# DCDmllm/AnyEdit

Hardware: AMD Instinct MI355X
Metric: edited-images/sec @512x512, 50 DDIM steps (higher is better)
Workload: dtype bf16; 1 GPU; configs[1]: AnySD (SD-1.5 UNet in=8 + task embedding/expert adapters) 512x512 bf16, 50 DDIM steps, batch=4/GPU, 3-branch CFG (UNet batch 12); images_per_gpu=4, ddim_steps=50, cfg_branches=3, hip_graph=True, parallelism=dp1 (image-sharded, no data-path collective)

## Files before the change

### anyedit_amd/_lib.py

```python
import ctypes
import os

import torch

_HERE = os.path.dirname(os.path.abspath(__file__))
LIB_PATH = os.environ.get("AE_LIB_PATH") or os.path.join(_HERE, "libanyedit_hip.so")

c_void_p, c_int, c_long, c_float = ctypes.c_void_p, ctypes.c_int, ctypes.c_long, ctypes.c_float

SIGNATURES = {
    "ae_version": [],
    "ae_last_error": [],
    "ae_device_arch": [ctypes.c_char_p, c_int],
    "ae_device_info": [ctypes.POINTER(c_int), ctypes.POINTER(c_long), ctypes.POINTER(c_int)],
    "ae_gemm_bf16": [c_void_p, c_long, c_void_p, c_long, c_int, c_void_p, c_long, c_void_p, c_long, c_int, c_int, c_int,
                     c_void_p, c_void_p, c_long, c_void_p, c_long, c_int, c_int, c_int, c_void_p, c_void_p],
    "ae_conv3x3_workspace_floats": [c_int, c_int, c_int, c_int, c_int, c_int, c_int],
    "ae_conv3x3_partials_bf16": [c_void_p, c_void_p, c_int, c_int, c_int, c_int, c_int, c_void_p, c_int, c_void_p, c_void_p],
    "ae_groupnorm_splitk_supported": [c_int, c_int, c_int, c_int, c_int],
    "ae_groupnorm_splitk_nhwc_bf16": [c_void_p, c_int, c_void_p, c_void_p, c_long, c_void_p, c_void_p, c_void_p, c_int, c_int, c_int, c_int, c_float, c_int, c_void_p],
    "ae_conv3x3_bf16": [c_void_p, c_void_p, c_void_p, c_void_p, c_long, c_void_p, c_void_p, c_int, c_int, c_int, c_int, c_int,
                        c_int, c_int, c_int, c_void_p, c_void_p, c_int, c_void_p],
    "ae_conv3x3_up2_bf16": [c_void_p, c_void_p, c_void_p, c_void_p, c_int, c_int, c_int, c_int, c_int, c_void_p, c_void_p],
    "ae_groupnorm_rows_per_chunk": [c_int, c_int],
    "ae_groupnorm_workspace_floats": [c_int, c_int, c_int, c_int],
    "ae_groupnorm_nhwc_bf16": [c_void_p, c_void_p, c_int, c_void_p, c_void_p, c_void_p, c_int, c_int, c_int, c_int, c_float,
                               c_int, c_void_p, c_void_p, c_void_p, c_void_p, c_void_p, c_void_p],
    "ae_layernorm_bf16": [c_void_p, c_void_p, c_void_p, c_void_p, c_int, c_int, c_float, c_void_p],
    "ae_attn_fwd_bf16": [c_void_p, c_void_p, c_void_p, c_void_p, c_int, c_int, c_int, c_int, c_int,
                         c_long, c_long, c_long, c_long, c_long, c_long, c_long, c_long, c_long, c_long, c_long, c_long,
                         c_float, c_void_p, c_void_p, c_int, c_int, c_void_p, c_void_p, c_int,
                         c_void_p, c_void_p, c_int, c_long, c_long, c_long, c_long, c_long, c_long, c_void_p, c_void_p, c_void_p,
                         c_void_p],
    "ae_attn_bwd_bf16": [c_void_p] * 10 + [c_int] * 5 + [c_long] * 21 + [c_float, c_void_p, c_int, c_void_p, c_void_p],
    "ae_attn_bwd_workspace_floats": [c_int] * 5,
    "ae_groupnorm_bwd_workspace_floats": [c_int, c_int, c_int, c_int],
    "ae_groupnorm_bwd_nhwc_bf16": [c_void_p, c_void_p, c_int, c_void_p, c_void_p, c_void_p, c_void_p, c_void_p, c_int, c_int, c_int,
                                   c_int, c_float, c_int, c_void_p, c_void_p, c_void_p, c_int, c_void_p],
    "ae_layernorm_bwd_bf16": [c_void_p, c_void_p, c_void_p, c_void_p, c_void_p, c_int, c_int, c_float, c_int, c_void_p],
    "ae_layernorm_param_grad_f32": [c_void_p, c_void_p, c_void_p, c_void_p, c_void_p, c_int, c_int, c_void_p],
    "ae_add_bf16": [c_void_p, c_void_p, c_void_p, c_long, c_void_p],
    "ae_axpy_bf16": [c_void_p, c_void_p, c_float, c_void_p, c_long, c_void_p],
    "ae_geglu_fwd_bf16": [c_void_p, c_void_p, c_long, c_int, c_void_p],
    "ae_geglu_bwd_bf16": [c_void_p, c_void_p, c_void_p, c_long, c_int, c_void_p],
    "ae_sumpool2x2_bf16": [c_void_p, c_void_p, c_int, c_int, c_int, c_int, c_void_p],
# ... 56 lines not shown
                             c_float, c_void_p],
    "ae_layernorm_act_bf16": [c_void_p, c_void_p, c_void_p, c_void_p, c_long, c_int, c_float, c_int, c_void_p],
    "ae_sam_pe_encode_f32": [c_void_p, c_void_p, c_void_p, c_void_p, c_void_p, c_int, c_int, c_float, c_float, c_float, c_void_p],
    "ae_sam_mask_downscale_bf16": [c_void_p] * 10 + [c_int, c_int, c_int, c_float, c_void_p],
    "ae_sam_mask_product_f32": [c_void_p, c_void_p, c_void_p, c_int, c_int, c_int, c_int, c_int, c_void_p],
    "ae_sam_postprocess_masks": [c_void_p, c_void_p, c_void_p] + [c_int] * 8 + [c_float, c_int, c_void_p],
    "ae_nms_sorted_f32": [c_void_p, c_void_p, c_int, c_float, c_void_p],
    "ae_sam_preprocess_f32": [c_void_p, c_int, c_void_p, c_int, c_int, c_int, c_int, c_int, c_void_p, c_void_p, c_void_p],
    "ae_patchify_f32_bf16": [c_void_p, c_void_p, c_int, c_int, c_int, c_int, c_int, c_void_p],
    "ae_mse_f32": [c_void_p, c_void_p, c_void_p, c_long, c_void_p],
    "ae_lincomb4_f32": [c_void_p, c_void_p, c_float, c_void_p, c_float, c_void_p, c_float, c_void_p, c_float, c_long, c_void_p],
    "ae_dpm_adaptive_err_f32": [c_void_p, c_void_p, c_void_p, c_float, c_float, c_int, c_long, c_void_p, c_void_p],
    "ae_task_gate": [c_void_p, c_void_p, c_void_p, c_void_p, c_int, c_int, c_int, c_int, c_void_p, c_void_p, c_void_p, c_void_p],
    "ae_attn_causal_short_bf16": [c_void_p, c_void_p, c_void_p, c_void_p, c_int, c_int, c_int, c_int] + [c_long] * 12 + [c_float, c_void_p],
    "ae_clip_embed_bf16": [c_void_p, c_int, c_void_p, c_void_p, c_void_p, c_int, c_int, c_int, c_int, c_int, c_void_p],
    "ae_bias_act_f32_bf16": [c_void_p, c_long, c_void_p, c_void_p, c_long, c_long, c_int, c_int, c_void_p],
    "ae_clip_pool_eos_bf16": [c_void_p, c_int, c_void_p, c_void_p, c_int, c_int, c_int, c_long, c_void_p],
    "ae_clip_patch_rows_bf16": [c_void_p, c_int, c_void_p, c_int, c_int, c_int, c_int, c_int, c_int, c_float, c_void_p, c_void_p, c_void_p],
    "ae_clip_vision_embed_ln_bf16": [c_void_p, c_long, c_void_p, c_void_p, c_void_p, c_void_p, c_void_p, c_int, c_int, c_int, c_float, c_void_p],
    "ae_clip_vision_pool_ln_bf16": [c_void_p, c_long, c_void_p, c_void_p, c_void_p, c_int, c_int, c_float, c_void_p],
    "ae_dino_embed_bf16": [c_void_p, c_long, c_void_p, c_void_p, c_void_p, c_void_p, c_int, c_int, c_int, c_void_p],
    "ae_swiglu_f32_bf16": [c_void_p, c_long, c_void_p, c_void_p, c_long, c_long, c_int, c_void_p],
}
_RESTYPES = {"ae_last_error": ctypes.c_char_p, "ae_groupnorm_workspace_floats": c_long, "ae_conv3x3_workspace_floats": c_long,
             "ae_groupnorm_bwd_workspace_floats": c_long, "ae_attn_fp8_workspace_bytes": c_long, "ae_attn_bwd_workspace_floats": c_long,
             "ae_xattn_fused_kv_bytes": c_long}


class AnyEditHipError(RuntimeError):
    pass


def _load():
    if not os.path.exists(LIB_PATH):
        raise ImportError(
            f"{LIB_PATH} is missing: the HIP extension is REQUIRED (no CPU/eager fallback exists). "
            "Build it with `python -c 'import __graft_entry__ as g; g.build()'` or `python anyedit_amd/build.py`.")
    lib = ctypes.CDLL(LIB_PATH)
    for name, argtypes in SIGNATURES.items():
        fn = getattr(lib, name)
        fn.argtypes = argtypes
        fn.restype = _RESTYPES.get(name, c_int)
    return lib


lib = _load()

# ... 12 lines not shown
```

### anyedit_amd/csrc/gemm_conv.hip

```cpp
#include "common.hpp"
#include <stdlib.h>
#include <type_traits>

namespace {

#ifndef AE_CONV_SPEC
#define AE_CONV_SPEC 1
#endif
#ifndef AE_GEMM_WA_DEFAULT
#define AE_GEMM_WA_DEFAULT 3
#endif
#ifndef AE_GEMM_PP_DEFAULT
#define AE_GEMM_PP_DEFAULT 63
#endif
#ifndef AE_XE_OCC
#define AE_XE_OCC 4
#endif
#ifndef AE_PP_LAB
#define AE_PP_LAB 0
#endif
#ifndef AE_PP_PRIO
#define AE_PP_PRIO 1
#endif
#ifndef AE_PP_DMA_FIRST
// ... 10 lines not shown
    const bf16_t* W;
    void* C;
    const float* bias;
    const bf16_t* res;
    const float* addvec;
    int M, N, K, Ksplit;
    long lda, lda2, ldw, ldc, ldr, ldav;
    int epi, out_f32, rows_per_batch;
    int H, Wd, Cin, CinPad, Ho, Wo, stride, ups;
    unsigned a_bytes, a2_bytes, w_bytes;
    int splitk;
    float* partial;
    float* colstats;
    int kmajor;
    int m_fast;
    int xe;
    float* rowstats;
    const float* ln_stats;
    const float* ln_colsum;
    int ln_parts;
    float ln_eps;
    int sub2;
    int defer_reduce;
};

__device__ __forceinline__ void lds_dma16(__amdgpu_buffer_rsrc_t rs, bf16_t* lds_dst, int voffset, int soffset = 0) {
#if defined(__HIP_DEVICE_COMPILE__)
    __builtin_amdgcn_raw_ptr_buffer_load_lds(rs, (__attribute__((address_space(3))) void*)lds_dst, 16, voffset, soffset, 0, 0);
#endif
}

#ifdef AE_GEMM_LAB
__device__ unsigned long long g_gemm_dbg[32];
#define GL_T(i) do { const unsigned long long t_ = __builtin_readcyclecounter(); if (lab_me) g_gemm_dbg[lab_base + (i)] += t_ - tlast; tlast = t_; } while (0)
#elif defined(AE_GEMM_TRACE)
constexpr int TR_K0 = 18, TR_T = 6;
__device__ unsigned long long g_pp_trace[8 * TR_T * 16];
#define GL_T(i) do { __builtin_amdgcn_sched_barrier(0); tr_t[(i)] = __builtin_readcyclecounter(); __builtin_amdgcn_sched_barrier(0); } while (0)
#else
#define GL_T(i)
#endif

constexpr int epilogue_passes(int FM, int bytes_per_frag_row, int lds_bytes) {
    for (int ps = 1; ps <= FM; ++ps)
        if (FM % ps == 0 && (FM / ps) * bytes_per_frag_row <= lds_bytes) return ps;
    return FM;
// ... 101 lines not shown
                for (int t9 = 0; t9 < 9; ++t9) {
                    const int iy = iy0 + t9 / 3, ix = ix0 + t9 % 3;
                    if ((unsigned)iy < (unsigned)Hv && (unsigned)ix < (unsigned)Wv && (p.ups != 2 || ((iy | ix) & 1) == 0)) fa_mask[i] |= 1u << t9;
                }
            }

        }
    }
#pragma unroll
    for (int i = 0; i < B_CH; ++i) {
        const int id = tid + i * NT, row = id >> 3;
        const int c = GLDS ? ((id & 7) ^ (row & 7)) : (id & 7);
        fb_off[i] = (n0 + row < p.N) ? (int)((long)(n0 + row) * p.ldw * 2) + c * 16 : OOB;
    }
    const bool conv_fast = (AMODE == A_CONV3) && p.Cin == p.CinPad;

    u32x4 ra[A_CH], rb[B_CH];
    const u32x4 zero4 = {0u, 0u, 0u, 0u};
    const int KT_all = (p.K + BK - 1) / BK;
    const int kt_per = (KT_all + p.splitk - 1) / p.splitk;
    const int kt_begin = (AMODE == A_CONV3 && p.sub2) ? 0 : split * kt_per;
    const int KT = max(min(KT_all - kt_begin, kt_per), 0);
    const int klast = p.K - 8;
    const int conv_per = AMODE == A_CONV3 ? p.CinPad / BK : 1;
    const unsigned conv_per_magic = (AE_CONV_SPEC && conv_per > 1) ? 0xFFFFFFFFu / (unsigned)conv_per + 1u : 0u;
    const unsigned pp_magic = (WA == 3 && conv_per > 1) ? 0xFFFFFFFFu / (unsigned)conv_per + 1u : 0u;
    int ld_tap = (kt_begin * BK) / (AMODE == A_CONV3 ? p.CinPad : 1 << 30), ld_ci = (AMODE == A_CONV3) ? (kt_begin * BK) % p.CinPad : 0;
    if (AMODE == A_CONV3 && p.kmajor) { ld_tap = kt_begin % 9; ld_ci = (kt_begin / 9) * BK; }

    auto load_tile = [&](int kt) __attribute__((always_inline)) {
        const int k0 = (kt_begin + kt) * BK;
        const bool full_k = k0 + BK <= p.K;
        if (AMODE == A_DENSE && full_k && (k0 + BK <= p.Ksplit || k0 >= p.Ksplit)) {
            if (k0 < p.Ksplit) {
#pragma unroll
                for (int i = 0; i < A_CH; ++i) ra[i] = __builtin_amdgcn_raw_buffer_load_b128(rsA, fa_off[i] + k0 * 2, 0, 0);
            } else {
#pragma unroll
                for (int i = 0; i < A_CH; ++i) ra[i] = __builtin_amdgcn_raw_buffer_load_b128(rsA2, fa2_off[i] + (k0 - p.Ksplit) * 2, 0, 0);
            }
#pragma unroll
            for (int i = 0; i < B_CH; ++i) rb[i] = __builtin_amdgcn_raw_buffer_load_b128(rsW, fb_off[i] + k0 * 2, 0, 0);
            return;
        }
        if (conv_fast) {
            const int ky = ld_tap / 3, kx = ld_tap - ky * 3;
// ... 168 lines not shown
        auto dma_a = [&](int kt, int buf) __attribute__((always_inline)) {
            const int fs = WA == 2 ? buf : 0;
            const int k0 = (kt_begin + kt) * BK;
            if (AMODE == A_DENSE) {
                const bool second = k0 >= p.Ksplit;
                if (AE_CONV_SPEC) {
                    if (!second) {
#pragma unroll
                        for (int i = 0; i < A_CH; ++i) lds_dma16(rsA, sA + buf * BM * BK + (wave + (NT / 64) * i) * 8 * BK, fa_off[i], k0 * 2);
                    } else {
#pragma unroll
                        for (int i = 0; i < A_CH; ++i) lds_dma16(rsA2, sA + buf * BM * BK + (wave + (NT / 64) * i) * 8 * BK, fa2_off[i], (k0 - p.Ksplit) * 2);
                    }
                } else {
#pragma unroll
                for (int i = 0; i < A_CH; ++i) {
                    bf16_t* dst = sA + buf * BM * BK + (wave + (NT / 64) * i) * 8 * BK;
                    if (!second) lds_dma16(rsA, dst, fa_off[i], k0 * 2);
                    else lds_dma16(rsA2, dst, fa2_off[i], (k0 - p.Ksplit) * 2);
                }
                }
            } else {
                constexpr bool KM1 = AE_CONV_SPEC && WA == 2;
                int cur_tap = ld_tap, cur_ci = ld_ci;
                constexpr bool STATELESS = true;
                if (STATELESS) {
                    const int lin = kt_begin + kt;
                    if (KM1 || p.kmajor) { cur_tap = lin % 9; cur_ci = (lin / 9) * BK; }
                    else if (AE_CONV_SPEC) {
                        cur_tap = conv_per == 1 ? lin : (int)__umulhi((unsigned)lin, conv_per_magic);
                        cur_ci = (lin - cur_tap * conv_per) * BK;
                    } else { const int per = p.CinPad / BK; cur_tap = lin / per; cur_ci = (lin - cur_tap * per) * BK; }
                }
                const int ky = (!KM1 && p.sub2) ? py + (cur_tap >> 1) : cur_tap / 3, kx = (!KM1 && p.sub2) ? px + (cur_tap & 1) : cur_tap - ky * 3;
                const int mbit = (!KM1 && p.sub2) ? ky * 3 + kx : cur_tap;
                if (cur_ci == 0 || kt == 0 || KM1 || p.kmajor || WA == 2) {
#pragma unroll
                    for (int i = 0; i < A_CH; ++i) {
                        int src = fa_off[i] + ((ky * p.Wd + kx) * p.Cin) * 2;
                        if (!KM1 && p.ups) {
                            const int cc = ((tid + i * NT) & 7) ^ (((tid + i * NT) >> 3) & 7);
                            src = (int)((a_base[i] + (long)(max(a_iy[i] + ky, 0) >> 1) * p.Wd + (max(a_ix[i] + kx, 0) >> 1)) * p.Cin + cc * 8) * 2;
                        }
                        fa_cur[fs][i] = ((fa_mask[i] >> mbit) & 1u) ? src : OOB;
                    }
                }
// ... 853 lines not shown
    hipLaunchKernelGGL(kern, dim3(grid), dim3(threads), lds, stream, a);
    return ae_check_launch(what);
}

template <int AMODE>
int launch(const GemmArgs& a_in, hipStream_t stream) {
    GemmArgs a = a_in;
    static const int mfast_env = getenv("AE_GEMM_MFAST") ? atoi(getenv("AE_GEMM_MFAST")) : -1;
    a.m_fast = mfast_env >= 0 ? mfast_env : (AMODE == A_CONV3 ? (9L * a.N >= 8L * a.M) : ((long)a.N >= 3L * a.M)) ? 1 : 0;
    const int cand[4][2] = {{128, 128}, {128, 64}, {64, 64}, {128, 160}};
    static const int t160 = getenv("AE_GEMM_T160") ? atoi(getenv("AE_GEMM_T160")) : 1;
    int pick = a.splitk > 1 ? 0 : pick_tile(a.M, a.N);
    static const int force_tile = getenv("AE_GEMM_TILE") ? atoi(getenv("AE_GEMM_TILE")) : -1;
    if (force_tile >= 0 && force_tile <= 2 && a.splitk <= 1) pick = force_tile;
    if (pick == 3 && (!t160 || AMODE == A_DENSE || a.epi == EPI_GEGLU || a.splitk > 1)) pick = 1;
    static const int w8 = getenv("AE_GEMM_W8") ? atoi(getenv("AE_GEMM_W8")) : 2;
    static const int wk_knob = getenv("AE_GEMM_WK") ? atoi(getenv("AE_GEMM_WK")) : 0;
    const int kt_block = ((a.K + BK - 1) / BK + a.splitk - 1) / a.splitk;
    const bool wk_env = wk_knob == 2 || (wk_knob == 1 && AMODE == A_CONV3 && kt_block >= 60);
    const bool conv = AMODE == A_CONV3;
    const char* what = conv ? "ae_conv3x3_bf16" : "ae_gemm_bf16";
    static const int glds_env = getenv("AE_GEMM_GLDS") ? atoi(getenv("AE_GEMM_GLDS")) : 1;
    const bool glds = glds_env && (conv ? (a.Cin == a.CinPad) : (a.K % BK == 0 && (!a.A2 || a.Ksplit % BK == 0)));
    if (conv && a.kmajor && !glds) { ae_set_error("%s: the chunk-major K order exists only in the LDS-DMA loader (AE_GEMM_GLDS=0 is set)", what); return AE_ERR_UNSUPPORTED; }
    auto lds_of = [](int bm, int bn, int st) { return (size_t)st * (bm + bn) * BK * sizeof(bf16_t); };
    auto lds_wa = [](int bm, int bn) { return (size_t)(2 * bm + 3 * bn) * BK * sizeof(bf16_t); };
    static const int wa = getenv("AE_GEMM_WA") ? atoi(getenv("AE_GEMM_WA")) : AE_GEMM_WA_DEFAULT;
#ifdef AE_GEMM_TRACE
    auto lds_aa = [](int bm, int bn) { return (size_t)(3 * bm + 2 * bn) * BK * sizeof(bf16_t) + 8192; };
#else
    auto lds_aa = [](int bm, int bn) { return (size_t)(3 * bm + 2 * bn) * BK * sizeof(bf16_t); };
#endif
    static const int pp = getenv("AE_GEMM_PP") ? atoi(getenv("AE_GEMM_PP")) : AE_GEMM_PP_DEFAULT;
    int rc = 0;

    static const int t320 = getenv("AE_GEMM_T320") ? atoi(getenv("AE_GEMM_T320")) : 11;
    bool done = false;
    bool xe_done = false;
    const bool cs_epi_ok = a.colstats && a.epi != EPI_GEGLU && !a.out_f32 && a.splitk <= 1 && a.N % 8 == 0 && a.ldc % 8 == 0 &&
                           (!a.res || (a.ldr % 8 == 0 && (reinterpret_cast<uintptr_t>(a.res) & 15) == 0));
    bool cs_done = false;
#ifdef AE_GEMM_ABLATE
    static const int lab_abl = getenv("AE_GEMM_ABL") ? atoi(getenv("AE_GEMM_ABL")) : 0;
#endif
    const bool slab_ok = conv && a.kmajor && a.stride == 1 && !a.ups && a.Cin == a.CinPad && a.H == a.Ho && a.Wd == a.Wo && a.Wd % 16 == 0 && 192 % a.Wd == 0 &&
                         192 / a.Wd <= a.H + 1 &&
                         (a.splitk <= 1 || kt_block % 9 == 0);
    const size_t lds_slab = (size_t)2 * ((192 + 192 / 16 + 1 + 7) / 8) * 1024 + (size_t)2 * 320 * BK * sizeof(bf16_t);
    if (conv && a.splitk > 1 && glds && make_plan(a.M, a.N, a.K, true).tile == 4) {
        const long t = (long)(a.M / 192) * (a.N / 320) * a.splitk;
        if ((pp & 32) && (pp & 2) && slab_ok) { if constexpr (AMODE == A_CONV3) rc = launch_kernel(gemm_kernel<192, 320, A_CONV3, 2, 4, true, 1, 2, false, 0, 4>, (unsigned)t, 512, lds_slab, stream, a, what); }
        else if ((pp & 2) && !a.ups) { if constexpr (AMODE == A_CONV3) rc = launch_kernel(gemm_kernel<192, 320, A_CONV3, 2, 4, true, 1, 2, false, 0, 3>, (unsigned)t, 512, lds_aa(192, 320), stream, a, what); }
        else rc = launch_kernel(gemm_kernel<192, 320, AMODE, 2, 4, true>, (unsigned)t, 512, lds_of(192, 320, 2), stream, a, what);
        done = true;
    }
    if (!done && t320 && glds && a.splitk <= 1 && a.N % 320 == 0 && ((conv && (t320 & 1)) || (!conv && a.epi == EPI_GEGLU && a.K >= 640 && (t320 & 2)) || (!conv && a.epi == EPI_GEGLU && a.K < 640 && a.K >= 320 && (t320 & 4)) ||
                                                                     (!conv && a.epi != EPI_GEGLU && a.K >= 640 && (t320 & 8)))) {
        const long t = (long)((a.M + 191) / 192) * (a.N / 320);
        const double fill = (double)t / (double)(((t + 255) / 256) * 256) * ((double)a.M / (double)(((a.M + 191) / 192) * 192));
        static const int t320_xe = getenv("AE_GEMM_T320_XE") ? atoi(getenv("AE_GEMM_T320_XE")) : 1;
        const long t128x = (long)((a.M + 127) / 128) * ((a.N + 127) / 128);
        const bool xe_tail = t320_xe && !conv && a.xe == 2 && a.epi != EPI_GEGLU && (pp & 8) && fill >= 0.74 && fill < 0.85 &&
                             (double)t128x / (double)(((t128x + 511) / 512) * 512) <= 0.72;
        if (fill >= 0.85 || xe_tail) {
            if (xe_tail) {
                if constexpr (AMODE == A_DENSE) { rc = launch_kernel(gemm_kernel<192, 320, A_DENSE, 4, 2, true, 1, 2, false, 0, 3, 2>, (unsigned)t, 512, lds_aa(192, 320) + 2 * 320 * sizeof(float), stream, a, what); xe_done = true; }
            } else
            if (a.epi == EPI_GEGLU && (pp & 8)) {
                if constexpr (AMODE == A_DENSE) {
                    if (a.xe == 2) { rc = launch_kernel(gemm_kernel<192, 320, A_DENSE, 4, 2, true, 1, 2, false, 0, 3, 2>, (unsigned)t, 512, lds_aa(192, 320) + 2 * 320 * sizeof(float), stream, a, what); xe_done = true; }
                    else rc = launch_kernel(gemm_kernel<192, 320, A_DENSE, 4, 2, true, 1, 2, false, 0, 3>, (unsigned)t, 512, lds_aa(192, 320), stream, a, what);
                }
            }
            else if (a.epi == EPI_GEGLU) rc = launch_kernel(gemm_kernel<192, 320, AMODE, 4, 2, true>, (unsigned)t, 512, lds_of(192, 320, 2), stream, a, what);
            else if (conv && (pp & 1) && !a.ups) {
                if constexpr (AMODE == A_CONV3) {
                    const bool slab = (pp & 16) && slab_ok;
                    if (slab && cs_epi_ok) { rc = launch_kernel(gemm_kernel<192, 320, A_CONV3, 2, 4, true, 1, 2, true, 0, 4>, (unsigned)t, 512, lds_slab, stream, a, what); cs_done = true; }
                    else if (slab) rc = launch_kernel(gemm_kernel<192, 320, A_CONV3, 2, 4, true, 1, 2, false, 0, 4>, (unsigned)t, 512, lds_slab, stream, a, what);
                    else if (cs_epi_ok) { rc = launch_kernel(gemm_kernel<192, 320, A_CONV3, 2, 4, true, 1, 2, true, 0, 3>, (unsigned)t, 512, lds_aa(192, 320), stream, a, what); cs_done = true; }
                    else rc = launch_kernel(gemm_kernel<192, 320, A_CONV3, 2, 4, true, 1, 2, false, 0, 3>, (unsigned)t, 512, lds_aa(192, 320), stream, a, what);
                }
            } else if (!conv && (pp & 4)) {
                if constexpr (AMODE == A_DENSE) rc = launch_kernel(gemm_kernel<192, 320, A_DENSE, 2, 4, true, 1, 2, false, 0, 3>, (unsigned)t, 512, lds_aa(192, 320), stream, a, what);
            } else if (cs_epi_ok && AMODE == A_CONV3) {
                if constexpr (AMODE == A_CONV3) rc = launch_kernel(gemm_kernel<192, 320, A_CONV3, 2, 4, true, 1, 2, true>, (unsigned)t, 512, lds_of(192, 320, 2), stream, a, what);
                cs_done = true;
// ... 289 lines not shown
    AE_REQUIRE(Cout % 4 == 0, "ae_conv3x3_bf16: Cout=%d must be a multiple of 4", Cout);
    AE_REQUIRE(stride == 1 || stride == 2, "ae_conv3x3_bf16: stride must be 1 or 2");
    AE_REQUIRE(upsample2x >= 0 && upsample2x <= 2, "ae_conv3x3_bf16: upsample2x must be 0, 1 (nearest) or 2 (zero-insert)");
    AE_REQUIRE(!(upsample2x && stride != 1), "ae_conv3x3_bf16: upsample2x requires stride 1");
    AE_REQUIRE(aligned16(x) && aligned16(w) && aligned16(y), "ae_conv3x3_bf16: pointers must be 16-byte aligned");
    const int Hv = upsample2x ? 2 * H : H, Wv = upsample2x ? 2 * W : W;
    const int Ho = (Hv + 2 - 3) / stride + 1, Wo = (Wv + 2 - 3) / stride + 1;
    GemmArgs a{};
    a.A = (const bf16_t*)x; a.A2 = nullptr; a.W = (const bf16_t*)w; a.C = y;
    a.bias = bias; a.res = (const bf16_t*)residual; a.addvec = addvec;
    const int CinPad = (Cin + BK - 1) / BK * BK;
    a.M = B * Ho * Wo; a.N = Cout; a.K = 9 * CinPad; a.Ksplit = a.K;
    a.lda = 0; a.lda2 = 0; a.ldw = 9L * CinPad; a.ldc = Cout; a.ldr = Cout; a.ldav = addvec_ld > 0 ? addvec_ld : Cout;
    a.epi = EPI_NONE; a.out_f32 = out_f32; a.rows_per_batch = Ho * Wo;
    a.H = H; a.Wd = W; a.Cin = Cin; a.CinPad = CinPad; a.Ho = Ho; a.Wo = Wo; a.stride = stride; a.ups = upsample2x;
    a.a_bytes = (unsigned)((long)B * H * W * Cin * 2); a.a2_bytes = 0u; a.w_bytes = (unsigned)((long)Cout * 9 * CinPad * 2);
    AE_REQUIRE((long)B * H * W * Cin * 2 < (1L << 31) && (long)Cout * 9 * CinPad * 2 < (1L << 31), "ae_conv3x3_bf16: operands must be smaller than 2 GiB");
    a.splitk = workspace ? make_plan(a.M, a.N, a.K, true).splitk : 1;
    a.partial = workspace;
    a.colstats = colstats;
    a.kmajor = k_order;
    return launch<A_CONV3>(a, (hipStream_t)stream);
}
```

### anyedit_amd/ldm/modules/diffusionmodules/openaimodel.py

```python
from abc import abstractmethod
import math

import torch
import torch.nn as nn

from anyedit_amd import ops
from anyedit_amd.ldm.util import exists
from anyedit_amd.ldm.modules.attention import SpatialTransformer
from anyedit_amd.ldm.modules.diffusionmodules.util import avg_pool_nd, conv_nd, linear, normalization, zero_module

BF16 = torch.bfloat16


class TimestepBlock(nn.Module):

    @abstractmethod
    def forward(self, x, emb):
        """Apply the module to `x` given `emb` timestep embeddings."""


class Feat:
    __slots__ = ("t", "B", "H", "W", "t2", "st", "st2")

    def __init__(self, t, B, H, W, t2=None, st=None, st2=None):
# ... 159 lines not shown
        h = self.in_layers[0].rows(f.t, B, H * W, silu=True, x2=f.t2, colstats=f.st, colstats2=f.st2)
        whole = (lambda: f.t if f.t2 is None else ops.concat_channels(f.t, f.t2))
        Ho, Wo, xs = H, W, None
        if self.up:
            Ho, Wo = 2 * H, 2 * W
            xs, _, _ = ops.resample2x_rows(whole(), B, H, W)
        elif self.down:
            h, Ho, Wo = ops.resample2x_rows(h, B, H, W, down=True)
            xs, _, _ = ops.resample2x_rows(whole(), B, H, W, down=True)
        conv1, norm2 = self.in_layers[2], self.out_layers[0]
        if not self.up and not ssn and ops.conv3x3_gn_splitk_ok(B, Ho, Wo, conv1.in_channels, self.out_channels, norm2.num_groups):
            g2, b2 = norm2._affine()
            h = ops.groupnorm_splitk(conv1.rows_partials(h, B, Ho, Wo), conv1.packed_bias(), emb_out, g2, b2, B, Ho * Wo, norm2.eps, silu=True, groups=norm2.num_groups)
        else:
            st1 = _stats_for(B, Ho, Wo, self.out_channels, dev)
            if self.up:
                h, _, _ = conv1.rows(h, B, H, W, addvec=None if ssn else emb_out, upsample2x=True, colstats=st1)
            else:
                h, _, _ = conv1.rows(h, B, Ho, Wo, addvec=None if ssn else emb_out, colstats=st1)
            if ssn:
                h = ops.scale_shift_rows(norm2.rows(h, B, Ho * Wo, silu=False, colstats=st1), emb_out, B, Ho * Wo, silu=True)
            else:
                h = norm2.rows(h, B, Ho * Wo, silu=True, colstats=st1)
        if isinstance(self.skip_connection, nn.Identity):
            res = whole() if xs is None else xs
        elif self.skip_connection.kernel_size[0] == 1 and xs is None:
            res, _, _ = self.skip_connection.rows(f.t, B, H, W, a2=f.t2)
        else:
            res, _, _ = self.skip_connection.rows(whole() if xs is None else xs, B, Ho, Wo)
        st = _stats_for(B, Ho, Wo, self.out_channels, dev)
        y, _, _ = self.out_layers[3].rows(h, B, Ho, Wo, residual=res, colstats=st)
        return Feat(y, B, Ho, Wo, st=st)

    def forward(self, x, emb):
        B, C, H, W = x.shape
        f = self.rows(Feat(ops.nchw_to_rows(x), B, H, W), ops.silu_to_bf16(emb))
        return ops.rows_to_nchw(f.t, B, f.H, f.W, out_dtype=x.dtype)

    _forward = forward


class _QKVAttentionBase(nn.Module):

    def __init__(self, n_heads):
        super().__init__()
        self.n_heads = n_heads

    def _offsets(self, ch):
        raise NotImplementedError

    def rows(self, qkv, B, T):
        width = qkv.shape[1]
        assert width % (3 * self.n_heads) == 0
        ch = width // (3 * self.n_heads)
        (oq, ok, ov), hs = self._offsets(ch)
# ... 270 lines not shown
```

### anyedit_amd/ops.py

```python
import torch

import ctypes
import os
import threading

from ._lib import lib, check as _check

BF16 = torch.bfloat16
EPI_NONE, EPI_GELU, EPI_GEGLU, EPI_SILU, EPI_RELU = 0, 1, 2, 3, 4


def _s():
    return torch.cuda.current_stream().cuda_stream


def _p(t):
    return None if t is None else t.data_ptr()


_live = threading.local()


def _tmp(t):
    if t is not None:
# ... 485 lines not shown
        raise ValueError(f"conv3x3: x must be contiguous [B*H*W, Cin] = [{B * H * W}, Cin], got {tuple(x.shape)}")
    if w.shape[1] != 9 * ((Cin + 63) // 64 * 64):
        raise ValueError(f"conv3x3: packed weight has K={w.shape[1]}, expected {9 * ((Cin + 63) // 64 * 64)}")
    Hv, Wv = (2 * H, 2 * W) if upsample2x else (H, W)
    Ho, Wo = (Hv - 1) // stride + 1, (Wv - 1) // stride + 1
    if out is None:
        out = torch.empty(B * Ho * Wo, Cout, dtype=torch.float32 if out_f32 else BF16, device=x.device)
    if residual is not None:
        _chk(residual, BF16, "conv3x3.residual", 2)
        if residual.shape != (B * Ho * Wo, Cout) or not residual.is_contiguous():
            raise ValueError("conv3x3: residual shape mismatch")
    nws = lib.ae_conv3x3_workspace_floats(B, H, W, Cin, Cout, stride, int(upsample2x))
    ws = torch.empty(nws, dtype=torch.float32, device=x.device) if nws > 0 else None
    if colstats is not None:
        _chk(colstats, torch.float32, "conv3x3.colstats", 3)
        if tuple(colstats.shape) != ((B * Ho * Wo + 31) // 32, Cout, 2) or not colstats.is_contiguous():
            raise ValueError(f"conv3x3: colstats must be a contiguous [{(B * Ho * Wo + 31) // 32}, {Cout}, 2] fp32 buffer")
    check(lib.ae_conv3x3_bf16(_p(x), _p(w), _p(bias), _p(addvec), addvec.stride(0) if addvec is not None else 0, _p(residual),
                              _p(out), B, H, W, Cin, Cout, stride, int(upsample2x), 1 if out_f32 else 0, _p(ws), _p(colstats), int(k_order), _s()),
          "ae_conv3x3_bf16")
    return out, Ho, Wo


_GN_SPLITK = os.environ.get("AE_GN_SPLITK", "0") == "1"


def conv3x3_gn_splitk_ok(B, H, W, Cin, Cout, groups=32):
    if not _GN_SPLITK or (_TAPE is not None and _TAPE.active) or H * W > 256 or Cin % 8 or Cout % 8:
        return False
    nws = lib.ae_conv3x3_workspace_floats(B, H, W, Cin, Cout, 1, 0)
    if nws <= 0:
        return False
    return bool(lib.ae_groupnorm_splitk_supported(B, H * W, Cout, groups, int(nws // (B * H * W * Cout))))


def conv3x3_partials(x, w, B, H, W, k_order=0):
    _no_tape("conv3x3_partials")
    _chk(x, BF16, "conv3x3_partials.x", 2)
    _chk(w, BF16, "conv3x3_partials.w", 2)
    Cin, Cout = x.shape[1], w.shape[0]
    if x.shape[0] != B * H * W or not x.is_contiguous() or w.shape[1] != 9 * ((Cin + 63) // 64 * 64):
        raise ValueError(f"conv3x3_partials: x [B*H*W, Cin] contiguous and w packed [Cout, 9*CinPad] expected, got {tuple(x.shape)} / {tuple(w.shape)}")
    nws = lib.ae_conv3x3_workspace_floats(B, H, W, Cin, Cout, 1, 0)
    if nws <= 0:
        raise ValueError(f"conv3x3_partials: the plan of [{B * H * W}, {Cin}] -> {Cout} does not cut K")
    ws = torch.empty(nws, dtype=torch.float32, device=x.device)
# ... 1139 lines not shown

def _up2_label(_r, x, w4, bias, B, H, W, **_):
    y = _r[0]
    M, Cout, Cin = x.shape[0], w4.shape[1], x.shape[1]
    t192 = (M // 192) * (Cout // 320) * 4 if (M % 192 == 0 and Cout % 320 == 0) else 0
    tl = "192x320" if t192 and t192 / (-(-t192 // 256) * 256) >= 0.85 else "128x128"
    nb = 2 * (x.numel() + 16 * Cin * Cout) + 2 * y.numel()
    return f"gemm_kernel<{tl},conv3x3,up2x2>|M={y.shape[0]} Cin={Cin} Cout={Cout}", 2.0 * y.shape[0] * Cout * 4 * Cin, float(nb)


conv3x3_up2 = _wrap_profiled(conv3x3_up2, _up2_label)
xattn_fused = _wrap_profiled(xattn_fused, lambda _r, x, gamma, beta, eps, wq_img, kv_img, gate, wo_img, bo, rows_per_sample, Nk, T, scale, out=None: (
    f"xattn_fused_kernel<C=320>|M={x.shape[0]} Nk={Nk}+{T}", 2.0 * x.shape[0] * 320 * (2 * 320 + 2 * (Nk + T)), float(2 * (3 * x.numel() + wq_img.numel() + wo_img.numel() + kv_img.numel()))))
ff_fused = _wrap_profiled(ff_fused, lambda _r, x, gamma, beta, eps, w1, b1, w2img, b2, residual=None, out=None, w3=None, b3=None, residual3=None, colstats=None: (
    f"ff_fused_kernel<C=320{',proj_out' if w3 is not None else ''}>|M={x.shape[0]} H={w1.shape[0] // 2}",
    2.0 * x.shape[0] * x.shape[1] * (3 * (w1.shape[0] // 2) + (x.shape[1] if w3 is not None else 0)),
    float(2 * (x.numel() * (2 + (residual is not None and residual is not x) + (residual3 is not None)) + w1.numel() + w2img.numel() + (w3.numel() if w3 is not None else 0))),
    2 if colstats is not None else 1))
_ln_gemm_fused = _wrap_profiled(_ln_gemm_launch, _ln_gemm_label)
_gemm_ln_launch = _wrap_profiled(_gemm_ln_launch, _gemm_ln_label)
gemm = _wrap_profiled(gemm, _gemm_label)
attention_fp8 = _wrap_profiled(attention_fp8, _attn8_label)
conv3x3 = _wrap_profiled(conv3x3, _conv_label)
conv3x3_partials = _wrap_profiled(conv3x3_partials, lambda _r, x, w, B, H, W, k_order=0: (
    f"gemm_kernel<{_tile_label(x.shape[0], w.shape[0], True, 9 * (-(-x.shape[1] // 64) * 64), False, x.shape[1] % 64 == 0)},conv3x3>|M={x.shape[0]} Cin={x.shape[1]} Cout={w.shape[0]} s1 partials",
    2.0 * x.shape[0] * w.shape[0] * 9 * x.shape[1], float(2 * (x.numel() + 9 * x.shape[1] * w.shape[0]) + 2 * x.shape[0] * w.shape[0]), 1))
groupnorm_splitk = _wrap_profiled(groupnorm_splitk, lambda _r, partials, *a, **k: (
    f"groupnorm(splitK fold)|rows={_r.shape[0]} C={_r.shape[1]}", 0.0, 2.0 * _r.numel() * 2, 1))
attention = _wrap_profiled(attention, _attn_label)
groupnorm = _wrap_profiled(groupnorm, _gn_label)
layernorm = _wrap_profiled(layernorm, _ln_label)
expert_kv = _wrap_profiled(expert_kv, lambda _r, x, W, experts, tokens: (
    f"expert_kv_fwd_kernel|rows={x.shape[0]} N={W.shape[1]} Dc={W.shape[2]}", 2.0 * x.shape[0] * W.shape[1] * W.shape[2], 4.0 * (x.shape[0] // tokens) * W.shape[1] * W.shape[2]))
expert_kv_dgrad = _wrap_profiled(expert_kv_dgrad, lambda _r, dy, W, experts, tokens: (
    f"expert_kv_dgrad_kernel|rows={dy.shape[0]} N={W.shape[1]} Dc={W.shape[2]}", 2.0 * dy.shape[0] * W.shape[1] * W.shape[2], 4.0 * (dy.shape[0] // tokens) * W.shape[1] * W.shape[2]))
expert_kv_wgrad = _wrap_profiled(expert_kv_wgrad, lambda _r, dy, x, experts, tokens, n_experts, out=None: (
    f"expert_kv_wgrad_kernel|rows={dy.shape[0]} N={dy.shape[1]} Dc={x.shape[1]} E={n_experts}", 2.0 * dy.shape[0] * dy.shape[1] * x.shape[1], 4.0 * n_experts * dy.shape[1] * x.shape[1]))
```

### include/anyedit_hip.h

```cpp
#ifndef ANYEDIT_HIP_H
#define ANYEDIT_HIP_H

#ifdef __cplusplus
extern "C" {
#endif

#define AE_OK 0
#define AE_ERR_ARG (-1)
#define AE_ERR_LAUNCH (-2)
#define AE_ERR_UNSUPPORTED (-3)

#define AE_EPI_NONE 0
#define AE_EPI_GELU 1
#define AE_EPI_GEGLU 2
#define AE_EPI_SILU 3
#define AE_EPI_RELU 4

int ae_version(void);
const char* ae_last_error(void);
int ae_device_arch(char* buf, int n);
int ae_device_info(int* cus, long* hbm_bytes, int* clock_khz);

int ae_gemm_bf16(const void* A, long lda, const void* A2, long lda2, int Ksplit, const void* W, long ldw, void* C, long ldc,
                 int M, int N, int K, const float* bias, const void* residual, long ldr, const float* addvec, long addvec_ld,
// ... 5 lines not shown
                    float* colstats , void* stream);

int ae_gemm_ln_plan(int M, int N, int K, int epilogue, int mode);
int ae_gemm_ln_bf16(const void* A, long lda, const void* W, long ldw, void* C, long ldc, int M, int N, int K, const float* bias,
                    const void* residual, long ldr, int epilogue, float* rowstats_out, const float* ln_stats, int ln_parts,
                    const float* ln_colsum, float ln_eps, void* stream);

int ae_ff_fused_supported(int M, int C, int H);
int ae_ff_fused_bf16(const void* X, long ldx, const float* ln_gamma, const float* ln_beta, float ln_eps, const void* W1, long ldw1, const float* b1,
                     const void* W2img, const float* b2, const void* residual, long ldr, const void* W3, long ldw3, const float* b3,
                     const void* residual3, long ldr3, float* colstats, void* Y, long ldy, int M, int C, int H, void* stream);

int ae_xattn_fused_supported(int M, int C, int heads, int head_dim, int rows_per_sample, int Nk, int T);
int ae_xattn_fused_covers(int M, int C, int heads, int head_dim, int rows_per_sample, int Nk, int T);
long ae_xattn_fused_kv_bytes(void);
int ae_xattn_fused_bf16(const void* X, long ldx, const float* ln_gamma, const float* ln_beta, float ln_eps, const void* Wq_img, const void* KV_img, const float* gate,
                        const void* Wo_img, const float* bo, void* Y, long ldy, int M, int rows_per_sample, int Nk, int T, float scale, void* stream);

long ae_conv3x3_workspace_floats(int B, int H, int W, int Cin, int Cout, int stride, int upsample2x);
int ae_conv3x3_partials_bf16(const void* x, const void* w, int B, int H, int W, int Cin, int Cout, float* workspace, int k_order, int* splitk_out, void* stream);
int ae_conv3x3_bf16(const void* x, const void* w, const float* bias, const float* addvec, long addvec_ld, const void* residual,
                    void* y, int B, int H, int W, int Cin, int Cout, int stride, int upsample2x, int out_f32, float* workspace,
                    float* colstats , int k_order, void* stream);

int ae_conv3x3_up2_bf16(const void* x, const void* w4, const float* bias, void* y, int B, int H, int W, int Cin, int Cout,
                        float* colstats, void* stream);

int ae_groupnorm_rows_per_chunk(int HW, int C);
long ae_groupnorm_workspace_floats(int B, int HW, int C, int groups);
int ae_groupnorm_splitk_supported(int B, int HW, int C, int groups, int splitk);
int ae_groupnorm_splitk_nhwc_bf16(const float* partial, int splitk, const float* bias, const float* addvec, long addvec_ld, const float* gamma, const float* beta,
                                  void* y, int B, int HW, int C, int groups, float eps, int act, void* stream);
 * colstats / colstats2: optional per-channel slab statistics of x / x2 as written by the kernels that PRODUCED them (the `colstats`
 * output of ae_gemm_bf16 / ae_ln_gemm_bf16 / ae_conv3x3_bf16: [B*HW/32][C1][2] and [B*HW/32][C-C1][2]; HW % 32 == 0).  With them the
 * statistics pass over the activation is skipped: one block per (sample, group) folds the slab sums, then the apply launch runs.    */
int ae_groupnorm_nhwc_bf16(const void* x, const void* x2, int C1, const float* gamma, const float* beta, void* y, int B, int HW,
                           int C, int groups, float eps, int act, float* workspace, int* counters, float* stat_out,
                           const float* colstats, const float* colstats2, void* stream);

int ae_layernorm_bf16(const void* x, const float* gamma, const float* beta, void* y, int M, int C, float eps, void* stream);

int ae_attn_fwd_bf16(const void* q, const void* k, const void* v, void* out, int B, int H, int Nq, int Nk, int D,
                     long q_sb, long q_sh, long q_sn, long k_sb, long k_sh, long k_sn, long v_sb, long v_sh, long v_sn,
                     long o_sb, long o_sh, long o_sn, float scale, const float* rel_h, const float* rel_w, int kH, int kW,
                     const unsigned char* key_mask, const float* out_scale, int accumulate, const void* k2, const void* v2,
                     int Nk2, long k2_sb, long k2_sh, long k2_sn, long v2_sb, long v2_sh, long v2_sn, const float* scale2,
// ... 131 lines not shown
```

Measured before the change: 6.711 edited-images/sec.

## Fold ResBlock 1x1 skip conv into the output 3x3 conv GEMM as extra K

Adds a conv3x3+skip kernel path that appends the 1x1 skip-connection input channels, possibly split across two concatenated tensors, as extra K tiles of the 3x3 conv implicit GEMM. The skip and conv weights are packed together and their biases summed. This removes the separate skip GEMM launch and the residual tensor round trip through memory in ResBlocks whose channel count changes. The fold is only taken when the plan supports it and never on the 192x320 tile plans, so some shapes may land on a less-tuned plan and the larger K may change split-K choices.

Result: no change. 6.727 edited-images/sec (median of 6 runs) (+0.2%).

```diff
diff --git a/anyedit_amd/_lib.py b/anyedit_amd/_lib.py
--- a/anyedit_amd/_lib.py
+++ b/anyedit_amd/_lib.py
@@ -21,6 +21,10 @@
     "ae_groupnorm_splitk_nhwc_bf16": [c_void_p, c_int, c_void_p, c_void_p, c_long, c_void_p, c_void_p, c_void_p, c_int, c_int, c_int, c_int, c_float, c_int, c_void_p],
     "ae_conv3x3_bf16": [c_void_p, c_void_p, c_void_p, c_void_p, c_long, c_void_p, c_void_p, c_int, c_int, c_int, c_int, c_int,
                         c_int, c_int, c_int, c_void_p, c_void_p, c_int, c_void_p],
+    "ae_conv3x3_skip_supported": [c_int] * 7,
+    "ae_conv3x3_skip_workspace_floats": [c_int] * 7,
+    "ae_conv3x3_skip_bf16": [c_void_p, c_void_p, c_void_p, c_void_p, c_long, c_void_p, c_void_p, c_int, c_int, c_void_p, c_int, c_int, c_int, c_int, c_int,
+                             c_int, c_int, c_int, c_void_p, c_void_p, c_int, c_void_p],
     "ae_conv3x3_up2_bf16": [c_void_p, c_void_p, c_void_p, c_void_p, c_int, c_int, c_int, c_int, c_int, c_void_p, c_void_p],
     "ae_groupnorm_rows_per_chunk": [c_int, c_int],
     "ae_groupnorm_workspace_floats": [c_int, c_int, c_int, c_int],
@@ -123,7 +127,7 @@
     "ae_dino_embed_bf16": [c_void_p, c_long, c_void_p, c_void_p, c_void_p, c_void_p, c_int, c_int, c_int, c_void_p],
     "ae_swiglu_f32_bf16": [c_void_p, c_long, c_void_p, c_void_p, c_long, c_long, c_int, c_void_p],
 }
-_RESTYPES = {"ae_last_error": ctypes.c_char_p, "ae_groupnorm_workspace_floats": c_long, "ae_conv3x3_workspace_floats": c_long,
+_RESTYPES = {"ae_last_error": ctypes.c_char_p, "ae_groupnorm_workspace_floats": c_long, "ae_conv3x3_workspace_floats": c_long, "ae_conv3x3_skip_workspace_floats": c_long,
              "ae_groupnorm_bwd_workspace_floats": c_long, "ae_attn_fp8_workspace_bytes": c_long, "ae_attn_bwd_workspace_floats": c_long,
              "ae_xattn_fused_kv_bytes": c_long}
 
diff --git a/anyedit_amd/csrc/gemm_conv.hip b/anyedit_amd/csrc/gemm_conv.hip
--- a/anyedit_amd/csrc/gemm_conv.hip
+++ b/anyedit_amd/csrc/gemm_conv.hip
@@ -56,6 +56,11 @@
     float ln_eps;
     int sub2;
     int defer_reduce;
+    const bf16_t* xs;
+    const bf16_t* xs2;
+    int sk_tiles, sk_c1;
+    int sk_ld1, sk_ld2;
+    unsigned xs_bytes, xs2_bytes;
 };
 
 __device__ __forceinline__ void lds_dma16(__amdgpu_buffer_rsrc_t rs, bf16_t* lds_dst, int voffset, int soffset = 0) {
@@ -203,6 +208,7 @@
     const int kt_begin = (AMODE == A_CONV3 && p.sub2) ? 0 : split * kt_per;
     const int KT = max(min(KT_all - kt_begin, kt_per), 0);
     const int klast = p.K - 8;
+    const int kt_skip0 = (AMODE == A_CONV3 && p.sk_tiles) ? KT_all - p.sk_tiles : 0x7fffffff;
     const int conv_per = AMODE == A_CONV3 ? p.CinPad / BK : 1;
     const unsigned conv_per_magic = (AE_CONV_SPEC && conv_per > 1) ? 0xFFFFFFFFu / (unsigned)conv_per + 1u : 0u;
     const unsigned pp_magic = (WA == 3 && conv_per > 1) ? 0xFFFFFFFFu / (unsigned)conv_per + 1u : 0u;
@@ -417,6 +423,22 @@
                 }
             } else {
                 constexpr bool KM1 = AE_CONV_SPEC && WA == 2;
+                if (kt_begin + kt >= kt_skip0) {
+                    const int c = kt_begin + kt - kt_skip0;
+                    const bool second = c >= p.sk_c1;
+                    const int ld2 = (second ? p.sk_ld2 : p.sk_ld1) * 2, koff = (second ? c - p.sk_c1 : c) * (BK * 2);
+                    const __amdgpu_buffer_rsrc_t rsS = __builtin_amdgcn_make_buffer_rsrc(const_cast<bf16_t*>(p.xs), 0, (int)p.xs_bytes, 0x00020000);
+                    const __amdgpu_buffer_rsrc_t rsS2 = __builtin_amdgcn_make_buffer_rsrc(const_cast<bf16_t*>(p.xs2 ? p.xs2 : p.xs), 0, (int)(p.xs2 ? p.xs2_bytes : 0u), 0x00020000);
+#pragma unroll
+                    for (int i = 0; i < A_CH; ++i) {
+                        const int id = tid + i * NT, row = id >> 3;
+                        const int off = (m0 + row < p.M) ? (m0 + row) * ld2 + (((id & 7) ^ (row & 7)) << 4) : OOB;
+                        bf16_t* dst = sA + buf * BM * BK + (wave + (NT / 64) * i) * 8 * BK;
+                        if (!second) lds_dma16(rsS, dst, off, koff);
+                        else lds_dma16(rsS2, dst, off, koff);
+                    }
+                    return;
+                }
                 int cur_tap = ld_tap, cur_ci = ld_ci;
                 constexpr bool STATELESS = true;
                 if (STATELESS) {
@@ -1316,6 +1338,8 @@
     const char* what = conv ? "ae_conv3x3_bf16" : "ae_gemm_bf16";
     static const int glds_env = getenv("AE_GEMM_GLDS") ? atoi(getenv("AE_GEMM_GLDS")) : 1;
     const bool glds = glds_env && (conv ? (a.Cin == a.CinPad) : (a.K % BK == 0 && (!a.A2 || a.Ksplit % BK == 0)));
+    const bool sk = conv && a.sk_tiles > 0;
+    if (sk && !glds) { ae_set_error("%s: the folded skip exists only in the LDS-DMA loader", what); return AE_ERR_UNSUPPORTED; }
     if (conv && a.kmajor && !glds) { ae_set_error("%s: the chunk-major K order exists only in the LDS-DMA loader (AE_GEMM_GLDS=0 is set)", what); return AE_ERR_UNSUPPORTED; }
     auto lds_of = [](int bm, int bn, int st) { return (size_t)st * (bm + bn) * BK * sizeof(bf16_t); };
     auto lds_wa = [](int bm, int bn) { return (size_t)(2 * bm + 3 * bn) * BK * sizeof(bf16_t); };
@@ -1342,6 +1366,7 @@
                          (a.splitk <= 1 || kt_block % 9 == 0);
     const size_t lds_slab = (size_t)2 * ((192 + 192 / 16 + 1 + 7) / 8) * 1024 + (size_t)2 * 320 * BK * sizeof(bf16_t);
     if (conv && a.splitk > 1 && glds && make_plan(a.M, a.N, a.K, true).tile == 4) {
+        if (sk) { ae_set_error("%s: the 192x320 split-K plan does not carry the folded skip (M=%d N=%d K=%d)", what, a.M, a.N, a.K); return AE_ERR_UNSUPPORTED; }
         const long t = (long)(a.M / 192) * (a.N / 320) * a.splitk;
         if ((pp & 32) && (pp & 2) && slab_ok) { if constexpr (AMODE == A_CONV3) rc = launch_kernel(gemm_kernel<192, 320, A_CONV3, 2, 4, true, 1, 2, false, 0, 4>, (unsigned)t, 512, lds_slab, stream, a, what); }
         else if ((pp & 2) && !a.ups) { if constexpr (AMODE == A_CONV3) rc = launch_kernel(gemm_kernel<192, 320, A_CONV3, 2, 4, true, 1, 2, false, 0, 3>, (unsigned)t, 512, lds_aa(192, 320), stream, a, what); }
@@ -1357,6 +1382,7 @@
         const bool xe_tail = t320_xe && !conv && a.xe == 2 && a.epi != EPI_GEGLU && (pp & 8) && fill >= 0.74 && fill < 0.85 &&
                              (double)t128x / (double)(((t128x + 511) / 512) * 512) <= 0.72;
         if (fill >= 0.85 || xe_tail) {
+            if (sk) { ae_set_error("%s: the 192x320 plan does not carry the folded skip (M=%d N=%d K=%d)", what, a.M, a.N, a.K); return AE_ERR_UNSUPPORTED; }
             if (xe_tail) {
                 if constexpr (AMODE == A_DENSE) { rc = launch_kernel(gemm_kernel<192, 320, A_DENSE, 4, 2, true, 1, 2, false, 0, 3, 2>, (unsigned)t, 512, lds_aa(192, 320) + 2 * 320 * sizeof(float), stream, a, what); xe_done = true; }
             } else
@@ -1692,3 +1718,70 @@
     a.kmajor = k_order;
     return launch<A_CONV3>(a, (hipStream_t)stream);
 }
+
+namespace {
+bool skip_args(GemmArgs& a, const void* x, const void* w, const void* xs, const void* xs2, int B, int H, int W, int Cin, int Cout, int Cs1, int Cs) {
+    if (B <= 0 || H <= 0 || W <= 0 || Cin <= 0 || Cout <= 0 || Cin % 64 || Cout % 4 || Cs1 <= 0 || Cs1 % 64 || Cs % 64 || Cs1 > Cs) return false;
+    const long M = (long)B * H * W, K = 9L * Cin + Cs;
+    if (M * Cin * 2 >= (1L << 31) || M * Cs1 * 2 >= (1L << 31) || M * (Cs - Cs1) * 2 >= (1L << 31) || (long)Cout * K * 2 >= (1L << 31)) return false;
+    a = GemmArgs{};
+    a.A = (const bf16_t*)x; a.W = (const bf16_t*)w;
+    a.M = (int)M; a.N = Cout; a.K = (int)K; a.Ksplit = a.K;
+    a.ldw = K; a.ldc = Cout; a.ldr = Cout; a.ldav = Cout;
+    a.epi = EPI_NONE; a.rows_per_batch = H * W;
+    a.H = H; a.Wd = W; a.Cin = Cin; a.CinPad = Cin; a.Ho = H; a.Wo = W; a.stride = 1; a.ups = 0;
+    a.a_bytes = (unsigned)(M * Cin * 2); a.w_bytes = (unsigned)((long)Cout * K * 2);
+    a.xs = (const bf16_t*)xs; a.xs2 = Cs1 < Cs ? (const bf16_t*)xs2 : nullptr;
+    a.sk_tiles = Cs / 64; a.sk_c1 = Cs1 / 64; a.sk_ld1 = Cs1; a.sk_ld2 = Cs - Cs1;
+    a.xs_bytes = (unsigned)(M * Cs1 * 2); a.xs2_bytes = (unsigned)(M * (Cs - Cs1) * 2);
+    a.splitk = make_plan(a.M, a.N, a.K, true).splitk;
+    return true;
+}
+int skip_plan_query(const GemmArgs& a) {
+    g_plan_query = 1;
+    const int rc = launch<A_CONV3>(a, nullptr);
+    g_plan_query = 0;
+    return rc;
+}
+}
+
+extern "C" int ae_conv3x3_skip_supported(int B, int H, int W, int Cin, int Cout, int Cs1, int Cs) {
+    GemmArgs a;
+    const void* stand_in = reinterpret_cast<const void*>(uintptr_t(256));
+    if (!skip_args(a, stand_in, stand_in, stand_in, stand_in, B, H, W, Cin, Cout, Cs1, Cs)) return 0;
+    a.C = const_cast<void*>(stand_in);
+    a.partial = reinterpret_cast<float*>(uintptr_t(256));
+    int r = 0;
+    for (int ko = 0; ko < 2; ++ko) {
+        a.kmajor = ko;
+        if (skip_plan_query(a) == 0) r |= 1 << ko;
+    }
+    return r;
+}
+
+extern "C" long ae_conv3x3_skip_workspace_floats(int B, int H, int W, int Cin, int Cout, int Cs1, int Cs) {
+    GemmArgs a;
+    const void* stand_in = reinterpret_cast<const void*>(uintptr_t(256));
+    if (!skip_args(a, stand_in, stand_in, stand_in, stand_in, B, H, W, Cin, Cout, Cs1, Cs)) return 0;
+    return a.splitk > 1 ? (long)a.splitk * a.M * Cout : 0;
+}
+
+extern "C" int ae_conv3x3_skip_bf16(const void* x, const void* w, const float* bias, const float* addvec, long addvec_ld,
+                                    const void* xs, const void* xs2, int Cs1, int Cs, void* y, int B, int H, int W, int Cin, int Cout, int stride, int upsample2x,
+                                    int out_f32, float* workspace, float* colstats, int k_order, void* stream) {
+    AE_REQUIRE(x && w && y && xs, "ae_conv3x3_skip_bf16: null pointer");
+    AE_REQUIRE(k_order == 0 || k_order == 1, "ae_conv3x3_skip_bf16: k_order must be 0 (tap, channel) or 1 (64-channel chunk, tap, channel)");
+    AE_REQUIRE(B > 0 && H > 0 && W > 0, "ae_conv3x3_skip_bf16: bad shape B=%d H=%d W=%d", B, H, W);
+    AE_REQUIRE(stride == 1 && !upsample2x, "ae_conv3x3_skip_bf16: the folded skip needs stride 1 and no upsampling");
+    AE_REQUIRE(Cin > 0 && Cin % 64 == 0 && Cout > 0 && Cout % 4 == 0, "ae_conv3x3_skip_bf16: Cin=%d must be a multiple of 64, Cout=%d a multiple of 4", Cin, Cout);
+    AE_REQUIRE(Cs1 > 0 && Cs1 % 64 == 0 && Cs % 64 == 0 && Cs1 <= Cs, "ae_conv3x3_skip_bf16: skip channels must be whole 64-channel chunks (Cs1=%d, Cs=%d)", Cs1, Cs);
+    AE_REQUIRE((Cs1 < Cs) == (xs2 != nullptr), "ae_conv3x3_skip_bf16: xs2 goes with Cs1 < Cs (Cs1=%d, Cs=%d)", Cs1, Cs);
+    AE_REQUIRE(aligned16(x) && aligned16(w) && aligned16(y) && aligned16(xs) && aligned16(xs2), "ae_conv3x3_skip_bf16: pointers must be 16-byte aligned");
+    if (colstats) AE_REQUIRE(!out_f32 && Cout % 8 == 0 && (reinterpret_cast<uintptr_t>(colstats) & 15) == 0, "ae_conv3x3_skip_bf16: column statistics need a bf16 output with Cout %% 8 == 0");
+    GemmArgs a;
+    AE_REQUIRE(skip_args(a, x, w, xs, xs2, B, H, W, Cin, Cout, Cs1, Cs), "ae_conv3x3_skip_bf16: operands must be smaller than 2 GiB");
+    AE_REQUIRE(workspace || a.splitk <= 1, "ae_conv3x3_skip_bf16: the plan cuts K %d ways: a workspace of ae_conv3x3_skip_workspace_floats() floats is required", a.splitk);
+    a.C = y; a.bias = bias; a.addvec = addvec; a.ldav = addvec_ld > 0 ? addvec_ld : Cout;
+    a.out_f32 = out_f32; a.partial = workspace; a.colstats = colstats; a.kmajor = k_order;
+    return launch<A_CONV3>(a, (hipStream_t)stream);
+}
diff --git a/anyedit_amd/ldm/modules/diffusionmodules/openaimodel.py b/anyedit_amd/ldm/modules/diffusionmodules/openaimodel.py
--- a/anyedit_amd/ldm/modules/diffusionmodules/openaimodel.py
+++ b/anyedit_amd/ldm/modules/diffusionmodules/openaimodel.py
@@ -205,6 +205,15 @@
                 h = ops.scale_shift_rows(norm2.rows(h, B, Ho * Wo, silu=False, colstats=st1), emb_out, B, Ho * Wo, silu=True)
             else:
                 h = norm2.rows(h, B, Ho * Wo, silu=True, colstats=st1)
+        skip = self.skip_connection
+        if not isinstance(skip, nn.Identity) and skip.kernel_size[0] == 1 and xs is None and not ssn and f.t.is_contiguous() and (f.t2 is None or f.t2.is_contiguous()):
+            Cs1 = f.t.shape[1]
+            ko = ops.conv3x3_skip_plan(B, H, W, self.out_channels, self.out_channels, Cs1, Cs1 + (f.t2.shape[1] if f.t2 is not None else 0))
+            if ko is not None:
+                w, b = self._skip_packed(ko)
+                st = _stats_for(B, H, W, self.out_channels, dev)
+                y, _, _ = ops.conv3x3_skip(h, w, b, B, H, W, f.t, f.t2, colstats=st, k_order=ko)
+                return Feat(y, B, H, W, st=st)
         if isinstance(self.skip_connection, nn.Identity):
             res = whole() if xs is None else xs
         elif self.skip_connection.kernel_size[0] == 1 and xs is None:
@@ -214,6 +223,14 @@
         st = _stats_for(B, Ho, Wo, self.out_channels, dev)
         y, _, _ = self.out_layers[3].rows(h, B, Ho, Wo, residual=res, colstats=st)
         return Feat(y, B, Ho, Wo, st=st)
+
+    def _skip_packed(self, k_order):
+        conv2, skip = self.out_layers[3], self.skip_connection
+        if ops.cache_stale(self, "_skip_pk", conv2.weight, conv2.bias, skip.weight, skip.bias):
+            self._skip_pk = {}
+        if k_order not in self._skip_pk:
+            self._skip_pk[k_order] = ops.pack_conv3x3_skip(conv2.weight, conv2.bias, skip.weight, skip.bias, k_order=k_order)
+        return self._skip_pk[k_order]
 
     def forward(self, x, emb):
         B, C, H, W = x.shape
diff --git a/anyedit_amd/ops.py b/anyedit_amd/ops.py
--- a/anyedit_amd/ops.py
+++ b/anyedit_amd/ops.py
@@ -531,6 +531,68 @@
     return out, Ho, Wo
 
 
+_SKIP_FOLD = os.environ.get("AE_SKIP_FOLD", "1") != "0"
+_SKIP_PLAN = {}
+
+
+def conv3x3_skip_plan(B, H, W, Cin, Cout, Cs1, Cs):
+    if not _SKIP_FOLD or _GN_SPLITK or (_TAPE is not None and _TAPE.active):
+        return None
+    key = (B, H, W, Cin, Cout, Cs1, Cs)
+    r = _SKIP_PLAN.get(key)
+    if r is None:
+        r = _SKIP_PLAN[key] = int(lib.ae_conv3x3_skip_supported(B, H, W, Cin, Cout, Cs1, Cs))
+    if not r:
+        return None
+    ko = conv_k_order(B * H * W, Cin, Cout)
+    return ko if (r >> ko) & 1 else None
+
+
+def pack_conv3x3_skip(w3, b3, w1, b1, k_order=0):
+    w = torch.cat([pack_conv3x3(w3, k_order=k_order), pack_linear(w1)], dim=1).contiguous()
+    bs = [b.detach().float() for b in (b3, b1) if b is not None]
+    return w, ((bs[0] + bs[1]) if len(bs) == 2 else bs[0]).contiguous() if bs else None
+
+
+def conv3x3_skip(x, w, bias, B, H, W, xs, xs2=None, addvec=None, out_f32=False, out=None, colstats=None, k_order=0, workspace=None):
+    _no_tape("conv3x3_skip")
+    _chk(x, BF16, "conv3x3_skip.x", 2)
+    _chk(w, BF16, "conv3x3_skip.w", 2)
+    _chk(xs, BF16, "conv3x3_skip.xs", 2)
+    M, Cin, Cout, Cs1 = B * H * W, x.shape[1], w.shape[0], xs.shape[1]
+    Cs = Cs1
+    if xs2 is not None:
+        _chk(xs2, BF16, "conv3x3_skip.xs2", 2)
+        Cs += xs2.shape[1]
+    if x.shape[0] != M or not x.is_contiguous() or xs.shape[0] != M or not xs.is_contiguous() or (xs2 is not None and (xs2.shape[0] != M or not xs2.is_contiguous())):
+        raise ValueError(f"conv3x3_skip: x, xs and xs2 must be contiguous [{M}, C] tensors, got {tuple(x.shape)}, {tuple(xs.shape)}, {None if xs2 is None else tuple(xs2.shape)}")
+    if tuple(w.shape) != (Cout, 9 * Cin + Cs) or not w.is_contiguous():
+        raise ValueError(f"conv3x3_skip: packed weight must be a contiguous [Cout, {9 * Cin + Cs}] tensor, got {tuple(w.shape)}")
+    if out is None:
+        out = torch.empty(M, Cout, dtype=torch.float32 if out_f32 else BF16, device=x.device)
+    if bias is not None:
+        _chk(bias, torch.float32, "conv3x3_skip.bias", 1)
+    if addvec is not None:
+        _chk(addvec, torch.float32, "conv3x3_skip.addvec", 2)
+    nws = lib.ae_conv3x3_skip_workspace_floats(B, H, W, Cin, Cout, Cs1, Cs)
+    ws = workspace
+    if ws is None:
+        ws = torch.empty(nws, dtype=torch.float32, device=x.device) if nws > 0 else None
+    elif nws > 0:
+        _chk(ws, torch.float32, "conv3x3_skip.workspace", 1)
+        if ws.numel() < nws or not ws.is_contiguous():
+            raise ValueError(f"conv3x3_skip: the workspace must hold {nws} contiguous fp32 elements")
+    else:
+        ws = None
+    if colstats is not None:
+        _chk(colstats, torch.float32, "conv3x3_skip.colstats", 3)
+        if tuple(colstats.shape) != ((M + 31) // 32, Cout, 2) or not colstats.is_contiguous():
+            raise ValueError(f"conv3x3_skip: colstats must be a contiguous [{(M + 31) // 32}, {Cout}, 2] fp32 buffer")
+    check(lib.ae_conv3x3_skip_bf16(_p(x), _p(w), _p(bias), _p(addvec), addvec.stride(0) if addvec is not None else 0, _p(xs), _p(xs2), Cs1, Cs,
+                                   _p(out), B, H, W, Cin, Cout, 1, 0, 1 if out_f32 else 0, _p(ws), _p(colstats), int(k_order), _s()), "ae_conv3x3_skip_bf16")
+    return out, H, W
+
+
 _GN_SPLITK = os.environ.get("AE_GN_SPLITK", "0") == "1"
 
 
@@ -1716,6 +1778,10 @@
 gemm = _wrap_profiled(gemm, _gemm_label)
 attention_fp8 = _wrap_profiled(attention_fp8, _attn8_label)
 conv3x3 = _wrap_profiled(conv3x3, _conv_label)
+conv3x3_skip = _wrap_profiled(conv3x3_skip, lambda _r, x, w, bias, B, H, W, xs, xs2=None, **_: (
+    f"gemm_kernel<{_tile_label(x.shape[0], w.shape[0], True, w.shape[1], False, True)},conv3x3+skip>|M={x.shape[0]} Cin={x.shape[1]} Cout={w.shape[0]} Cs={w.shape[1] - 9 * x.shape[1]} s1",
+    2.0 * x.shape[0] * w.shape[0] * w.shape[1], float(2 * (x.numel() + xs.numel() + (xs2.numel() if xs2 is not None else 0) + w.numel()) + _r[0].numel() * _r[0].element_size()),
+    2 if "splitK" in _tile_label(x.shape[0], w.shape[0], True, w.shape[1], False, True) else 1))
 conv3x3_partials = _wrap_profiled(conv3x3_partials, lambda _r, x, w, B, H, W, k_order=0: (
     f"gemm_kernel<{_tile_label(x.shape[0], w.shape[0], True, 9 * (-(-x.shape[1] // 64) * 64), False, x.shape[1] % 64 == 0)},conv3x3>|M={x.shape[0]} Cin={x.shape[1]} Cout={w.shape[0]} s1 partials",
     2.0 * x.shape[0] * w.shape[0] * 9 * x.shape[1], float(2 * (x.numel() + 9 * x.shape[1] * w.shape[0]) + 2 * x.shape[0] * w.shape[0]), 1))
diff --git a/include/anyedit_hip.h b/include/anyedit_hip.h
--- a/include/anyedit_hip.h
+++ b/include/anyedit_hip.h
@@ -51,6 +51,12 @@
 int ae_conv3x3_bf16(const void* x, const void* w, const float* bias, const float* addvec, long addvec_ld, const void* residual,
                     void* y, int B, int H, int W, int Cin, int Cout, int stride, int upsample2x, int out_f32, float* workspace,
                     float* colstats , int k_order, void* stream);
+
+int ae_conv3x3_skip_supported(int B, int H, int W, int Cin, int Cout, int Cs1, int Cs);
+long ae_conv3x3_skip_workspace_floats(int B, int H, int W, int Cin, int Cout, int Cs1, int Cs);
+int ae_conv3x3_skip_bf16(const void* x, const void* w, const float* bias, const float* addvec, long addvec_ld, const void* xs, const void* xs2, int Cs1, int Cs,
+                         void* y, int B, int H, int W, int Cin, int Cout, int stride, int upsample2x, int out_f32, float* workspace, float* colstats, int k_order,
+                         void* stream);
 
 int ae_conv3x3_up2_bf16(const void* x, const void* w4, const float* bias, void* y, int B, int H, int W, int Cin, int Cout,
                         float* colstats, void* stream);
```
